# Jun-CEN/Open-World-Semantic-Segmentation

Hardware: AMD Instinct MI355X
Metric: images/sec train-step, DeepLabV3+R101 768x768 bs=16; % HBM & MFMA roofline (higher is better)
Workload: dtype f16x2

## Files before the change

include/dmlnet_hip.h:

```cpp
#ifndef DMLNET_HIP_H
#define DMLNET_HIP_H

#include <stdint.h>

#ifdef __cplusplus
extern "C" {
#endif

#define DML_ABI_VERSION 6

enum { DML_F32 = 0, DML_BF16 = 1 };
enum { DML_EINVAL = -1, DML_EALIGN = -2, DML_EUNSUPPORTED = -3 };

int dml_abi_version(void);
const char* dml_target_arch(void);

typedef struct DmlConvDesc {
    const void* x;
    const void* w;
    void* y;
    const float* bias;
    float* stats;
    int32_t B, Hi, Wi, C, ldx;
    int32_t Ho, Wo, N, ldy;
// ... 106 lines not shown
                    float* scale, float* shift, float* save_mean, float* save_invstd, void* stream);
int dml_bn_moments(float* partials, int64_t M, int N, int stat_rows, double* moments, void* stream);
int dml_bn_finalize_moments(const double* moments, int ranks, int64_t M_each, int N, const float* gamma,
                            const float* beta, float* running_mean, float* running_var, float momentum,
                            float eps, float* scale, float* shift, float* save_mean, float* save_invstd,
                            void* stream);
int dml_bn_bwd_sums(float* partials, int nblocks, int N, double* sums, float* dgamma, float* dbeta,
                    void* stream);
int dml_bn_bwd_coef(const double* sums, int64_t M_total, int N, const float* gamma, const float* save_mean,
                    const float* save_invstd, float* coef, void* stream);
int dml_bn_stats(const void* y, float* partials, int64_t M, int N, int ldy, int dtype, void* stream);
int dml_bn_eval_coeffs(const float* gamma, const float* beta, const float* running_mean,
                       const float* running_var, float eps, float* scale, float* shift, int N,
                       void* stream);
typedef struct DmlBnEvalDesc {
    const float* gamma; const float* beta; const float* running_var; float* scale; float* shift;
    int32_t N; float eps;
} DmlBnEvalDesc;
int dml_bn_eval_coeffs_table(const DmlBnEvalDesc* table, int count, void* stream);
int dml_bn_apply(const void* y, const void* res, void* z, const float* scale, const float* shift,
                 const float* mean, uint8_t* mask, int64_t M, int N, int ldy, int ldres, int ldz, int relu,
                 int dtype, float drop_p, uint64_t drop_seed, float* amax, void* planes, int64_t plane_stride,
                 int32_t ldp, const float* unscale, int64_t res_plane_stride, const float* res_unscale, void* stream);
int dml_bn_bwd_reduce(const void* dz, const void* y, const void* z, const uint8_t* mask, const float* save_mean,
                      const float* save_invstd, float* partials, int64_t M, int N, int lddz, int ldy,
                      int ldz, int relu, float gscale, int dtype, int* nblocks, float* gmax, void* stream);
int dml_bn_bwd_finalize(float* partials, int nblocks, int64_t M, int N, const float* gamma,
                        const float* save_mean, const float* save_invstd, float* dgamma, float* dbeta,
                        float* coef, void* stream);
int dml_bn_bwd_apply(const void* dz, const void* y, const void* z, const uint8_t* mask, const float* coef, void* dy,
                     void* dres, int64_t M, int N, int lddz, int ldy, int ldz, int lddy, int lddres,
                     int relu, float gscale, int dres_accum, int dtype, float* amax, void* planes, int64_t plane_stride,
                     int32_t ldp, const float* unscale, void* stream);
int dml_h2_bound_bn(const float* gamma, const float* beta, int N, int64_t count, float mult, const float* res_amax,
                    float* work, void* stream);
int dml_h2_bound_bn_bwd(const float* coef, const float* save_invstd, int N, int64_t count, const float* g_amax,
                        float* work, void* stream);
int dml_bn_finalize_bound(float* partials, int64_t M, int N, int stat_rows, const float* gamma, const float* beta,
                          float* running_mean, float* running_var, float momentum, float eps,
                          float* scale, float* shift, float* save_mean, float* save_invstd,
                          int64_t count, float mult, const float* res_amax, float* work, uint32_t* state, void* stream);
int dml_bn_bwd_finalize_bound(float* partials, int nblocks, int64_t M, int N, const float* gamma,
                              const float* save_mean, const float* save_invstd, float* dgamma, float* dbeta,
                              float* coef, int64_t count, const float* g_amax, float* work, uint32_t* state, void* stream);
typedef struct DmlH2BoundDesc {
    const float* gamma;
    const float* beta;
    float* work;
    int32_t N;
    float root_count, mult;
    int32_t reserved;
} DmlH2BoundDesc;
int dml_h2_bound_bn_table(const DmlH2BoundDesc* table_device, int count, void* stream);
int dml_h2_bound_bn_multi(const DmlH2BoundDesc* table_device, int count, float* work, void* stream);

int dml_maxpool3x3s2_fwd(const void* x, void* y, uint8_t* argmax, int B, int H, int W, int C, int dtype,
                         void* stream);
int dml_maxpool3x3s2_bwd(const void* dy, const uint8_t* argmax, void* dx, int B, int H, int W, int C,
                         int dtype, void* stream);
int dml_global_avgpool_fwd(const void* x, void* y, int B, int HW, int C, int ldx, int dtype, void* stream);
int dml_broadcast_hw(const void* v, void* z, int B, int HW, int C, int ldz, int dtype, void* stream);
int dml_reduce_hw(const void* dz, void* dv, int B, int HW, int C, int lddz, int dtype, void* stream);
int dml_reduce_hw_f32(const void* x, float* out, int B, int HW, int C, int ldx, int dtype, float scale, void* stream);
int dml_avgpool_bwd_add(const void* dv, void* dx, int B, int HW, int C, int lddx, int dtype, void* stream);
int dml_avgpool_bwd_set(const void* dv, void* dx, int B, int HW, int C, int lddx, int dtype, void* stream);

// ... 127 lines not shown
```

open-world-semantic-segmentation_amd/csrc/bn.hip:

```cpp
#include "common.h"
#include <cstdlib>

namespace {

struct Moments {
    double n, mean, m2;
};
__device__ __forceinline__ void merge(Moments& a, double nb, double meanb, double m2b) {
    if (nb <= 0.0) return;
    const double n = a.n + nb;
    const double d = meanb - a.mean;
    a.mean += d * (nb / n);
    a.m2 += m2b + d * d * (a.n * nb / n);
    a.n = n;
}

constexpr int FIN_CH = 4, FIN_SL = 64;
__device__ __forceinline__ double shfl_xor_f64(double v, int mask) {
    const long long b = __double_as_longlong(v);
    const int lo = __shfl_xor((int)(b & 0xffffffffll), mask), hi = __shfl_xor((int)(b >> 32), mask);
    return __longlong_as_double(((long long)hi << 32) | (unsigned int)lo);
}

__device__ __forceinline__ float h2_words_max(const float* __restrict__ words, float* sh4) {
// ... 647 lines not shown
                    rb[u] = *reinterpret_cast<const float4*>(dres + m * lddres + c + 4);
                }
            }
        }
#pragma unroll
        for (int u = 0; u < U; ++u) {
            const int64_t m = m0 + (int64_t)u * RB;
            if (m >= r1) continue;
            float g[V] = {ga[u].x, ga[u].y, ga[u].z, ga[u].w, gb[u].x, gb[u].y, gb[u].z, gb[u].w};
            const float yy[V] = {ya[u].x, ya[u].y, ya[u].z, ya[u].w, yb[u].x, yb[u].y, yb[u].z, yb[u].w};
#pragma unroll
            for (int q = 0; q < V; ++q) {
                const bool on = ((bits[u] >> (q + (q >= 4 ? 4 : 0))) & 1u) != 0;
                g[q] = on ? g[q] : 0.f;
            }
            h8 hi, lo;
#pragma unroll
            for (int q = 0; q < V; ++q) {
                const float o = cA[q] * g[q] + cB[q] * (yy[q] - cM[q]) + cC[q];
                const float xs = o * h2s;
                const _Float16 h = (_Float16)xs;
                hi[q] = h;
                lo[q] = (_Float16)(xs - (float)h);
            }
            *reinterpret_cast<h8*>(planes + m * ldp + c) = hi;
            *reinterpret_cast<h8*>(planes + plane_stride + m * ldp + c) = lo;
            if (dres != nullptr) {
                float r[V] = {0.f, 0.f, 0.f, 0.f, 0.f, 0.f, 0.f, 0.f};
                if (dres_accum) { r[0] = ra[u].x; r[1] = ra[u].y; r[2] = ra[u].z; r[3] = ra[u].w; r[4] = rb[u].x; r[5] = rb[u].y; r[6] = rb[u].z; r[7] = rb[u].w; }
#pragma unroll
                for (int q = 0; q < V; ++q) r[q] += g[q] * gscale;
                *reinterpret_cast<float4*>(dres + m * lddres + c) = make_float4(r[0], r[1], r[2], r[3]);
                *reinterpret_cast<float4*>(dres + m * lddres + c + 4) = make_float4(r[4], r[5], r[6], r[7]);
            }
        }
    }
}

constexpr int FIN2_MAXCHUNK = 128;
__global__ __launch_bounds__(256) void bn_fold_partials_kernel(float* partials, int64_t G, int N, int R, int NC,
                                                               int last_rows, const int SR) {
    __shared__ double sh[3][4][64];
    const int c = threadIdx.x & 63, rl = threadIdx.x >> 6;
    const int n = blockIdx.x * 64 + c;
    const int64_t g0 = (int64_t)blockIdx.y * R;
    const int64_t g1 = (int)blockIdx.y == NC - 1 ? G : g0 + R;
    double S = 0.0, Q = 0.0, P = 0.0;
    if (n < N)
        #pragma unroll 8
        for (int64_t g = g0 + rl; g < g1; g += 4) {
            const float2 p = *reinterpret_cast<const float2*>(partials + (g * N + n) * 2);
            const double rows = g == G - 1 ? (double)last_rows : (double)SR;
            S += (double)p.x;
            Q += (double)p.y;
            P += (double)p.x * (double)p.x / rows;
        }
    sh[0][rl][c] = S;
    sh[1][rl][c] = Q;
    sh[2][rl][c] = P;
    __syncthreads();
    if (rl < 3 && n < N) {
        const double v = sh[rl][0][c] + sh[rl][1][c] + sh[rl][2][c] + sh[rl][3][c];
        reinterpret_cast<double*>(partials)[(g0 + rl) * N + n] = v;
    }
}

// ... 298 lines not shown
extern "C" int dml_bn_finalize_moments(const double* moments, int ranks, int64_t M_each, int N, const float* gamma,
                                       const float* beta, float* running_mean, float* running_var, float momentum,
                                       float eps, float* scale, float* shift, float* save_mean, float* save_invstd,
                                       void* stream) {
    if (!moments || !scale || !shift || !save_mean || ranks <= 0 || M_each <= 0 || N <= 0) return DML_EINVAL;
    hipLaunchKernelGGL(bn_finalize_moments_kernel, dim3((N + 255) / 256), dim3(256), 0, static_cast<hipStream_t>(stream),
                       moments, ranks, M_each, N, gamma, beta, running_mean, running_var, momentum, eps, scale, shift,
                       save_mean, save_invstd);
    DML_LAUNCH_CHECK();
    return 0;
}

extern "C" int dml_bn_bwd_sums(float* partials, int nblocks, int N, double* sums, float* dgamma, float* dbeta,
                               void* stream) {
    if (!partials || !sums || nblocks <= 0 || N <= 0) return DML_EINVAL;
    hipStream_t st = static_cast<hipStream_t>(stream);
    const int stride = fold_bwd_partials(partials, nblocks, N, st);
    hipLaunchKernelGGL(bn_bwd_finalize_kernel, dim3((N + FIN_CH - 1) / FIN_CH), dim3(256), 0, st, partials, nblocks,
                       (int64_t)1, N, (const float*)nullptr, (const float*)nullptr, (const float*)nullptr, dgamma, dbeta,
                       (float*)nullptr, sums, stride);
    DML_LAUNCH_CHECK();
    return 0;
}

extern "C" int dml_bn_bwd_coef(const double* sums, int64_t M_total, int N, const float* gamma, const float* save_mean,
                               const float* save_invstd, float* coef, void* stream) {
    if (!sums || !save_mean || !save_invstd || !coef || M_total <= 0 || N <= 0) return DML_EINVAL;
    hipLaunchKernelGGL(bn_bwd_coef_kernel, dim3((N + 255) / 256), dim3(256), 0, static_cast<hipStream_t>(stream), sums,
                       M_total, N, gamma, save_mean, save_invstd, coef);
    DML_LAUNCH_CHECK();
    return 0;
}

extern "C" int dml_bn_bwd_apply(const void* dz, const void* y, const void* z, const uint8_t* mask, const float* coef, void* dy,
                                void* dres, int64_t M, int N, int lddz, int ldy, int ldz, int lddy, int lddres,
                                int relu, float gscale, int dres_accum, int dtype, float* amax, void* planes,
                                int64_t plane_stride, int32_t ldp, const float* unscale, void* stream) {
    if (!dz || !y || !coef || (!dy && !planes) || M <= 0 || N <= 0) return DML_EINVAL;
    if (relu && !z && !mask) return DML_EINVAL;
    if (!vec_ok(dtype, N) || !vec_ok(dtype, lddz) || !vec_ok(dtype, ldy) || (dy && !vec_ok(dtype, lddy)) ||
        (relu && !mask && !vec_ok(dtype, ldz)) || (dres && !vec_ok(dtype, lddres)))
        return DML_EALIGN;
    if (M >= (1ll << 31)) return DML_EINVAL;
    if (planes) {
        if (dtype != DML_F32 || !unscale || plane_stride <= 0 || ldp < N) return DML_EINVAL;
        if ((ldp & 3) || (plane_stride & 3) || (reinterpret_cast<uintptr_t>(planes) & 7)) return DML_EALIGN;
    }
    const int V = dtype == DML_BF16 ? 8 : 4;
    hipStream_t st = static_cast<hipStream_t>(stream);
    constexpr int bt = 64;
    if (dtype == DML_F32 && planes && !dy && !amax && (mask || !relu) && (N & 7) == 0 && (lddz & 3) == 0 && (ldy & 3) == 0 &&
        (ldp & 7) == 0 && (plane_stride & 7) == 0 && (!dres || (lddres & 3) == 0) &&
        ((reinterpret_cast<uintptr_t>(planes) | reinterpret_cast<uintptr_t>(dz) | reinterpret_cast<uintptr_t>(y) |
          reinterpret_cast<uintptr_t>(dres)) & 15) == 0 && (reinterpret_cast<uintptr_t>(mask) & 1) == 0) {
        const ColGeom g8 = col_geom(M, N / 8, 2, stream_blocks(M, N, dtype), bt);
        hipLaunchKernelGGL((bn_bwd_apply_planes8_kernel<2>), dim3(g8.row_blocks, g8.col_chunks), dim3(bt), 0, st, (const float*)dz,
                           (const float*)y, mask, coef, (float*)dres, M, N, lddz, ldy, lddres, relu, gscale, dres_accum, g8.CB, g8.RB,
                           g8.rows_per_block, static_cast<_Float16*>(planes), plane_stride, (int)ldp, unscale);
        DML_LAUNCH_CHECK();
        return 0;
    }
    const ColGeom g = col_geom(M, N / V, 2, stream_blocks(M, N, dtype), bt);
    dim3 grid(g.row_blocks, g.col_chunks);
    if (dtype == DML_BF16)
        hipLaunchKernelGGL((bn_bwd_apply_cols_kernel<bf16_t, 2>), grid, dim3(bt), 0, st, (const bf16_t*)dz,
                           (const bf16_t*)y, (const bf16_t*)z, mask, coef, (bf16_t*)dy, (bf16_t*)dres, M, N, lddz, ldy,
                           ldz, lddy, lddres, relu, gscale, dres_accum, g.CB, g.RB, g.rows_per_block,
                           reinterpret_cast<uint32_t*>(amax), (_Float16*)nullptr, (int64_t)0, 0, (const float*)nullptr);
    else
        hipLaunchKernelGGL((bn_bwd_apply_cols_kernel<float, 2>), grid, dim3(bt), 0, st, (const float*)dz,
                           (const float*)y, (const float*)z, mask, coef, (float*)dy, (float*)dres, M, N, lddz, ldy, ldz,
                           lddy, lddres, relu, gscale, dres_accum, g.CB, g.RB, g.rows_per_block, reinterpret_cast<uint32_t*>(amax),
                           static_cast<_Float16*>(planes), plane_stride, (int)ldp, unscale);
    DML_LAUNCH_CHECK();
    return 0;
}

namespace {
__global__ __launch_bounds__(256) void h2_bound_kernel(const float* __restrict__ p0, const float* __restrict__ p1,
                                                       const float* __restrict__ p2, const float* __restrict__ invstd, int N,
                                                       float root_count, float mult, const float* __restrict__ words,
                                                       float* __restrict__ work, int bwd) {
    __shared__ float sh[4];
    __shared__ uint32_t shw[4];
    uint32_t wm = 0;
    if (words != nullptr)
        for (int i = threadIdx.x; i < 1024; i += 256) wm = max(wm, __float_as_uint(words[i]));
#pragma unroll
    for (int o = 32; o > 0; o >>= 1) wm = max(wm, (uint32_t)__shfl_xor((int)wm, o, 64));
    if ((threadIdx.x & 63) == 0) shw[threadIdx.x >> 6] = wm;
    __syncthreads();
    const float wmax = __uint_as_float(max(max(shw[0], shw[1]), max(shw[2], shw[3])));
    float b = 0.f;
    for (int n = threadIdx.x; n < N; n += 256) {
        float v;
        if (!bwd) v = fabsf(p0 ? p0[n] : 1.f) * root_count + fabsf(p1 ? p1[n] : 0.f);
        else v = fabsf(p0[n]) * wmax + fabsf(p1[n]) * root_count / invstd[n] + fabsf(p2[n]);
        b = fmaxf(b, v);
    }
#pragma unroll
    for (int o = 32; o > 0; o >>= 1) b = fmaxf(b, __shfl_xor(b, o, 64));
    if ((threadIdx.x & 63) == 0) sh[threadIdx.x >> 6] = b;
    __syncthreads();
    if (threadIdx.x != 0) return;
    b = fmaxf(fmaxf(sh[0], sh[1]), fmaxf(sh[2], sh[3]));
    b = bwd ? b : b * mult + wmax;
    b *= 1.0009765625f;
    const uint32_t m = __float_as_uint(b);
    float s = 1.0f;
    if (m != 0) {
// ... 88 lines not shown
```

open-world-semantic-segmentation_amd/csrc/plan_exec.hip:

```cpp
#include "common.h"

#include <cstring>
#include <tuple>
#include <utility>

namespace {

template <class T> struct Unpack {
    static T get(uint64_t w) {
        if constexpr (std::is_pointer<T>::value) {
            return reinterpret_cast<T>(static_cast<uintptr_t>(w));
        } else if constexpr (std::is_same<T, float>::value) {
            const uint32_t lo = (uint32_t)w;
            float f;
            std::memcpy(&f, &lo, 4);
            return f;
        } else if constexpr (std::is_same<T, double>::value) {
            double d;
            std::memcpy(&d, &w, 8);
            return d;
        } else {
            return static_cast<T>(static_cast<int64_t>(w));
        }
    }
// ... 12 lines not shown
struct Entry {
    const char* name;
    int (*run)(const uint64_t*, void*);
    int nargs;
};

#define DML_ENTRY(fn) {#fn, [](const uint64_t* w, void* st) -> int { return thunk_call(&fn, w, st); }, arity(&fn)}

const Entry kEntries[] = {
    DML_ENTRY(dml_conv_igemm),
    DML_ENTRY(dml_conv_wgrad),
    DML_ENTRY(dml_conv_wgrad_group),
    DML_ENTRY(dml_prep_weight),
    DML_ENTRY(dml_prep_weights),
    DML_ENTRY(dml_unpad_wgrad),
    DML_ENTRY(dml_bias_grad),
    DML_ENTRY(dml_bias_grad_ws),
    DML_ENTRY(dml_pack_input),
    DML_ENTRY(dml_pack_input_s2d),
    DML_ENTRY(dml_s2d_weights),
    DML_ENTRY(dml_s2d_wgrad),
    DML_ENTRY(dml_bn_finalize),
    DML_ENTRY(dml_bn_moments),
    DML_ENTRY(dml_bn_finalize_moments),
    DML_ENTRY(dml_bn_bwd_sums),
    DML_ENTRY(dml_bn_bwd_coef),
    DML_ENTRY(dml_bn_stats),
    DML_ENTRY(dml_bn_eval_coeffs),
    DML_ENTRY(dml_bn_eval_coeffs_table),
    DML_ENTRY(dml_bn_apply),
    DML_ENTRY(dml_bn_bwd_reduce),
    DML_ENTRY(dml_bn_bwd_finalize),
    DML_ENTRY(dml_bn_bwd_apply),
    DML_ENTRY(dml_maxpool3x3s2_fwd),
    DML_ENTRY(dml_maxpool3x3s2_bwd),
    DML_ENTRY(dml_global_avgpool_fwd),
    DML_ENTRY(dml_broadcast_hw),
    DML_ENTRY(dml_reduce_hw),
    DML_ENTRY(dml_reduce_hw_f32),
    DML_ENTRY(dml_avgpool_bwd_add),
    DML_ENTRY(dml_avgpool_bwd_set),
    DML_ENTRY(dml_bilinear_fwd),
    DML_ENTRY(dml_bilinear_bwd),
    DML_ENTRY(dml_proto_dist_fwd),
    DML_ENTRY(dml_upsample_dist_fwd),
    DML_ENTRY(dml_proto_dist_bwd),
    DML_ENTRY(dml_head_bwd_fused),
    DML_ENTRY(dml_argmax_msp),
    DML_ENTRY(dml_dissum_score),
    DML_ENTRY(dml_novel_relabel),
    DML_ENTRY(dml_loss_fwd),
    DML_ENTRY(dml_loss_finalize),
    DML_ENTRY(dml_loss_bwd),
    DML_ENTRY(dml_sgd_step),
    DML_ENTRY(dml_fill_f32),
    DML_ENTRY(dml_convert_dtype),
    DML_ENTRY(dml_adaptive_avgpool_fwd),
    DML_ENTRY(dml_proto_dist_nhwc),
    DML_ENTRY(dml_upsample_nhwc_to_nchw),
    DML_ENTRY(dml_confusion_update),
    DML_ENTRY(dml_class_feature_sum),
    DML_ENTRY(dml_label_encode),
    DML_ENTRY(dml_h2_split),
    DML_ENTRY(dml_h2_bound_bn),
    DML_ENTRY(dml_h2_bound_bn_bwd),
    DML_ENTRY(dml_h2_bound_bn_table),
// ... 97 lines not shown
```

open-world-semantic-segmentation_amd/dmlnet/_lib.py:

```python
from __future__ import annotations

import ctypes as C
import os

_HERE = os.path.dirname(os.path.abspath(__file__))
LIB_PATH = os.environ.get("DML_LIB_PATH") or os.path.join(_HERE, "libdmlnet_hip.so")

DML_F32, DML_BF16 = 0, 1
STAT_ROWS = 64
LOSS_BLOCKS = 2048

c_p = C.c_void_p
c_i = C.c_int
c_i64 = C.c_int64
c_f = C.c_float


class ConvDesc(C.Structure):
    _fields_ = [("x", c_p), ("w", c_p), ("y", c_p), ("bias", c_p), ("stats", c_p),
                ("B", C.c_int32), ("Hi", C.c_int32), ("Wi", C.c_int32), ("C", C.c_int32), ("ldx", C.c_int32),
                ("Ho", C.c_int32), ("Wo", C.c_int32), ("N", C.c_int32), ("ldy", C.c_int32),
                ("R", C.c_int32), ("S", C.c_int32), ("stride", C.c_int32), ("dil", C.c_int32),
                ("pad", C.c_int32), ("dtype", C.c_int32), ("y_f32", C.c_int32), ("accum", C.c_int32),
                ("mode", C.c_int32),
# ... 73 lines not shown
_PROTOS = {
    "dml_abi_version": (c_i, []),
    "dml_target_arch": (C.c_char_p, []),
    "dml_conv_igemm": (c_i, [C.POINTER(ConvDesc), c_p]),
    "dml_conv_stat_rows": (c_i, [C.POINTER(ConvDesc)]),
    "dml_h2_split_table": (c_i, [c_p, c_i, c_p]),
    "dml_h2_split": (c_i, [c_p, c_i64, c_i, c_i, c_p, c_i64, c_i, c_i, c_p, c_i, c_p]),
    "dml_conv_wgrad": (c_i, [C.POINTER(WgradDesc), c_p]),
    "dml_prep_weight": (c_i, [c_p, c_p, c_p, c_i, c_i, c_i, c_i, c_i, c_p]),
    "dml_prep_weights": (c_i, [c_p, c_i, c_i, c_p]),
    "dml_unpad_wgrad": (c_i, [c_p, c_p, c_i, c_i, c_i, c_i, c_p]),
    "dml_bias_grad": (c_i, [c_p, c_p, c_i64, c_i, c_i, c_i, c_p]),
    "dml_bias_grad_ws": (c_i, [c_p, c_p, c_i64, c_i, c_i, c_i, c_p, c_i64, c_p]),
    "dml_pack_input": (c_i, [c_p, c_p, c_i, c_i, c_i, c_i, c_i, c_i, c_p]),
    "dml_pack_input_s2d": (c_i, [c_p, c_p, c_i, c_i, c_i, c_i, c_p]),
    "dml_s2d_weights": (c_i, [c_p, c_p, c_i, c_i, c_i, c_p]),
    "dml_s2d_wgrad": (c_i, [c_p, c_p, c_i, c_i, c_i, c_p]),
    "dml_gather_taps": (c_i, [c_p, c_p, c_i, c_i, c_i, c_i, c_i, c_i, c_i, c_i, c_p]),
    "dml_bn_finalize": (c_i, [c_p, c_i64, c_i, c_i, c_p, c_p, c_p, c_p, c_f, c_f, c_p, c_p, c_p, c_p, c_p]),
    "dml_bn_moments": (c_i, [c_p, c_i64, c_i, c_i, c_p, c_p]),
    "dml_bn_finalize_moments": (c_i, [c_p, c_i, c_i64, c_i, c_p, c_p, c_p, c_p, c_f, c_f, c_p, c_p, c_p, c_p, c_p]),
    "dml_bn_bwd_sums": (c_i, [c_p, c_i, c_i, c_p, c_p, c_p, c_p]),
    "dml_bn_bwd_coef": (c_i, [c_p, c_i64, c_i, c_p, c_p, c_p, c_p, c_p]),
    "dml_bn_stats": (c_i, [c_p, c_p, c_i64, c_i, c_i, c_i, c_p]),
    "dml_bn_eval_coeffs": (c_i, [c_p, c_p, c_p, c_p, c_f, c_p, c_p, c_i, c_p]),
    "dml_bn_eval_coeffs_table": (c_i, [c_p, c_i, c_p]),
    "dml_bn_apply": (c_i, [c_p, c_p, c_p, c_p, c_p, c_p, c_p, c_i64, c_i, c_i, c_i, c_i, c_i, c_i, c_f, C.c_uint64, c_p,
                           c_p, c_i64, c_i, c_p, c_i64, c_p, c_p]),
    "dml_bn_bwd_reduce": (c_i, [c_p, c_p, c_p, c_p, c_p, c_p, c_p, c_i64, c_i, c_i, c_i, c_i, c_i, c_f, c_i,
                                C.POINTER(c_i), c_p, c_p]),
    "dml_bn_bwd_finalize": (c_i, [c_p, c_i, c_i64, c_i, c_p, c_p, c_p, c_p, c_p, c_p, c_p]),
    "dml_bn_bwd_apply": (c_i, [c_p, c_p, c_p, c_p, c_p, c_p, c_p, c_i64, c_i, c_i, c_i, c_i, c_i, c_i, c_i, c_f,
                               c_i, c_i, c_p, c_p, c_i64, c_i, c_p, c_p]),
    "dml_h2_bound_bn": (c_i, [c_p, c_p, c_i, c_i64, c_f, c_p, c_p, c_p]),
    "dml_h2_bound_bn_table": (c_i, [c_p, c_i, c_p]),
    "dml_h2_bound_bn_multi": (c_i, [c_p, c_i, c_p, c_p]),
    "dml_bilinear_fwd_planes": (c_i, [c_p, c_p, c_i64, c_i, c_p, c_i, c_i, c_i, c_i, c_i, c_i, c_i, c_p]),
    "dml_h2_bound_bn_bwd": (c_i, [c_p, c_p, c_i, c_i64, c_p, c_p, c_p]),
    "dml_bn_finalize_bound": (c_i, [c_p, c_i64, c_i, c_i, c_p, c_p, c_p, c_p, c_f, c_f, c_p, c_p, c_p, c_p,
                                    c_i64, c_f, c_p, c_p, c_p, c_p]),
    "dml_bn_bwd_finalize_bound": (c_i, [c_p, c_i, c_i64, c_i, c_p, c_p, c_p, c_p, c_p, c_p, c_i64, c_p, c_p, c_p, c_p]),
    "dml_maxpool3x3s2_fwd": (c_i, [c_p, c_p, c_p, c_i, c_i, c_i, c_i, c_i, c_p]),
    "dml_maxpool3x3s2_bwd": (c_i, [c_p, c_p, c_p, c_i, c_i, c_i, c_i, c_i, c_p]),
    "dml_global_avgpool_fwd": (c_i, [c_p, c_p, c_i, c_i, c_i, c_i, c_i, c_p]),
    "dml_broadcast_hw": (c_i, [c_p, c_p, c_i, c_i, c_i, c_i, c_i, c_p]),
    "dml_reduce_hw": (c_i, [c_p, c_p, c_i, c_i, c_i, c_i, c_i, c_p]),
    "dml_reduce_hw_f32": (c_i, [c_p, c_p, c_i, c_i, c_i, c_i, c_i, c_f, c_p]),
    "dml_avgpool_bwd_add": (c_i, [c_p, c_p, c_i, c_i, c_i, c_i, c_i, c_p]),
    "dml_avgpool_bwd_set": (c_i, [c_p, c_p, c_i, c_i, c_i, c_i, c_i, c_p]),
    "dml_bilinear_fwd": (c_i, [c_p, c_p, c_i, c_i, c_i, c_i, c_i, c_i, c_i, c_i, c_i, c_i, c_i, c_p]),
    "dml_bilinear_bwd": (c_i, [c_p, c_p, c_i, c_i, c_i, c_i, c_i, c_i, c_i, c_i, c_i, c_i, c_i, c_p]),
    "dml_proto_dist_fwd": (c_i, [c_p, c_p, c_p, c_p, c_p, c_p, c_i, c_i, c_i, c_i, c_i, c_p]),
    "dml_upsample_dist_fwd": (c_i, [c_p, c_p, c_p, c_p, c_p, c_p, c_i, c_i, c_i, c_i, c_i, c_i, c_i, c_p]),
    "dml_proto_dist_bwd": (c_i, [c_p, c_p, c_p, c_p, c_p, c_i, c_i, c_i, c_i, c_i, c_p]),
    "dml_head_bwd_fused": (c_i, [c_p, c_p, c_p, c_p, c_p, c_p, c_i, c_i, c_i, c_i, c_i, c_i, c_i, c_i64, c_f, c_f, c_i, c_p]),
    "dml_argmax_msp": (c_i, [c_p, c_p, c_p, c_i, c_i, c_i, c_i, c_p]),
    "dml_dissum_score": (c_i, [c_p, c_p, c_p, c_i, c_i, c_i, c_i, c_f, c_i, c_p]),
    "dml_novel_relabel": (c_i, [c_p, c_p, c_p, c_p, c_i, c_i, c_i, c_i, c_i, c_f, c_i64, c_p]),
    "dml_loss_fwd": (c_i, [c_p, c_p, c_p, c_p, c_i, c_i, c_i, c_i, c_i64, c_p]),
    "dml_loss_finalize": (c_i, [c_p, c_p, c_f, c_f, c_p]),
    "dml_loss_bwd": (c_i, [c_p, c_p, c_p, c_p, c_p, c_i, c_i, c_i, c_i, c_i64, c_f, c_f, c_p]),
    "dml_sgd_step": (c_i, [c_p, c_p, c_p, c_i64, c_f, c_f, c_f, c_f, c_p]),
    "dml_fill_f32": (c_i, [c_p, c_i64, c_f, c_p]),
    "dml_convert_dtype": (c_i, [c_p, c_p, c_i64, c_i, c_i, c_p]),
    "dml_confusion_update": (c_i, [c_p, c_p, c_p, c_i64, c_i, c_p]),
    "dml_class_feature_sum": (c_i, [c_p, c_p, c_i64, c_i, c_i64, c_p, c_p, c_p]),
# ... 60 lines not shown
```

open-world-semantic-segmentation_amd/dmlnet/engine.py:

```python
from __future__ import annotations

import ctypes as C
import itertools
import os
import struct
import weakref
from typing import List, Optional

import numpy as np
import torch
import torch.distributed as dist
import torch.nn as nn

from . import _lib, lazy_grad
from ._lib import DML_BF16, DML_F32, STAT_ROWS, ConvDesc, WgradDesc

_PAD_CIN = 8


class _S2DConv:

    def __init__(self, conv: nn.Conv2d, Ho: int, Wo: int):
        k, p = conv.kernel_size[0], conv.padding[0]
        self.real, self.k = conv, k
# ... 828 lines not shown
            sp = part.data_ptr()
        else:
            sp = self.sp
            a1 = self.call(self.bwd, lib.dml_bn_bwd_reduce, dz.ptr, u.y.ptr, u.z.ptr, mk, u.mean.data_ptr(),
                           u.invstd.data_ptr(), self.sp, M, N, dz.ld, u.y.ld, u.z.ld, 1 if relu_eff else 0, 1.0,
                           self.dt, C.byref(nblk), gwork.data_ptr() if gwork is not None else None)
        if self.sync and not u.frozen:
            sums = self.dbuf(N * 2)
            self.call(self.bwd, lib.dml_bn_bwd_sums, sp, nblk, N, sums.data_ptr(), st.grad_ptr_of(bn.weight),
                      st.grad_ptr_of(bn.bias))
            grp = self.e.sync_group
            self.py_op(self.bwd, lambda t=sums, g=grp: dist.all_reduce(t, group=g))
            self.call(self.bwd, lib.dml_bn_bwd_coef, sums.data_ptr(), M * self.world, N, bn.weight.data_ptr(),
                      u.mean.data_ptr(), u.invstd.data_ptr(), coef.data_ptr())
        elif dy_direct and self.fuse_bound:
            self.call(self.bwd, lib.dml_bn_bwd_finalize_bound, sp, nblk, 0 if u.frozen else M, N, bn.weight.data_ptr(),
                      u.mean.data_ptr(), u.invstd.data_ptr(), st.grad_ptr_of(bn.weight),
                      st.grad_ptr_of(bn.bias), coef.data_ptr(), M * self.world, gwork.data_ptr(), dy.h2[1].data_ptr(),
                      self.bound_state())
            bound_done = True
        else:
            self.call(self.bwd, lib.dml_bn_bwd_finalize, sp, nblk, 0 if u.frozen else M, N, bn.weight.data_ptr(),
                      u.mean.data_ptr(), u.invstd.data_ptr(), st.grad_ptr_of(bn.weight),
                      st.grad_ptr_of(bn.bias), coef.data_ptr())
        self.mark_grad(bn.weight)
        self.mark_grad(bn.bias)
        pl = (None, 0, 0, None)
        if dy_direct:
            planes, work = dy.h2
            if not bound_done:
                self.call(self.bwd, lib.dml_h2_bound_bn_bwd, coef.data_ptr(), u.invstd.data_ptr(), N, M * self.world,
                          gwork.data_ptr(), work.data_ptr())
            pl = (planes.data_ptr(), M * N, N, work.data_ptr() + 4096)
        a3 = self.call(self.bwd, lib.dml_bn_bwd_apply, dz.ptr, u.y.ptr, u.z.ptr, mk, coef.data_ptr(),
                       None if only else dy.ptr, dres.ptr if dres is not None else None, M, N, dz.ld, u.y.ld, u.z.ld, dy.ld,
                       dres.ld if dres is not None else 0, 1 if relu_eff else 0, 1.0,
                       1 if dres_accum else 0, self.dt, None if dy_direct else self.amax_of(dy), *pl)
        u.gscale_slots += ([(a1, 13)] if a1 is not None else []) + [(a3, 15)]
        if dres is not None:
            self.last_dgrad.pop(dres.ptr, None)
        self.conv_wgrad(u.x, dy, u.conv, u.Cp)
        if need_dgrad:
            self.conv_dgrad(dy, u.conv, u.wt, u.x, final=final)

    def block_fwd(self, x: Act, blk: nn.Module, out_planes_only=False):
        n1, n2, n3 = blk.conv1.out_channels, blk.conv2.out_channels, blk.conv3.out_channels
        kk = blk.conv2.kernel_size[0] * blk.conv2.kernel_size[1]
        u1 = self.cbr(x, blk.conv1, blk.bn1, planes_only=self.h2_ok(n1, n2, kk))
        u2 = self.cbr(u1.z, blk.conv2, blk.bn2, planes_only=self.h2_ok(n2, n3, 1))
        ud = None
        if blk.downsample is not None:
            ud = self.cbr(x, blk.downsample[0], blk.downsample[1], relu=False)
            idt = ud.z
        else:
            idt = x
        u3 = self.cbr(u2.z, blk.conv3, blk.bn3, relu=True, res=idt, planes_only=out_planes_only)
        return (x, u1, u2, u3, ud)

    def block_bwd(self, rec):
        xb, u1, u2, u3, ud = rec
        dz = self.grad_of(u3.z)
        ud_from_dz = False
        if ud is not None:
            ud_from_dz = (self.ds_grad_from_dz and u3.relu and u3.mask is not None and u3.drop is None and not ud.relu
                          and ud.drop is None and ud.z is ud.z.root and ud.conv.out_channels == u3.conv.out_channels)
            if ud_from_dz:
                self.unit_bwd(u3, dz, dres=None)
            else:
                dres = self.grad_of(ud.z)
                self.unit_bwd(u3, dz, dres=dres, dres_accum=False)
                ud.z.grad_init = True
        elif (self.fuse_res_grad and not xb.root.grad_init and xb is xb.root
              and u3.relu and u3.mask is not None and u3.drop is None and xb.C % 8 == 0 and xb.C > 32
              and dz.ld == xb.C and self.conv_geom(u1.conv, xb)[:3] == (1, 1, 1)
              and (self.dtype == torch.bfloat16
# ... 216 lines not shown
    def _head_bwd(self, rec, low: Act, out: Act):
        lib, st = self.lib, self.e.store
        B, H, W = self.B, self.H, self.W
        K, Kp, emb, fin, wt_fin = rec.K, rec.Kp, rec.emb, rec.fin, rec.wt_fin
        cat1, cat2, up_low, branches, pooled, upool = rec.cat1, rec.cat2, rec.up_low, rec.branches, rec.pooled, rec.upool
        uproj, ucls = rec.uproj, rec.ucls
        df = self.fbuf(B * H * W * Kp)
        rec.df = df
        de = self.new(B, emb.H, emb.W, Kp)
        rec.de = de
        rec.fused_args, rec.fused_range = None, None
        if Kp == 16 and K == 16 and H == 4 * emb.H and W == 4 * emb.W:
            i0 = len(self.bwd)
            rec.fused_args = self.call(self.bwd, lib.dml_head_bwd_fused, 0, 0, 0, 0, rec.protos.data_ptr(), de.ptr, B,
                                       emb.H, emb.W, Kp, K, H, W, 255, 0.0, 1.0, self.dt)
            rec.fused_range = (i0, i0 + 1)
        i1 = len(self.bwd)
        rec.head_bwd_args = self.call(self.bwd, lib.dml_proto_dist_bwd, 0, None, 0, rec.protos.data_ptr(),
                                       df.data_ptr(), B, Kp, K, H, W)
        self.call(self.bwd, lib.dml_bilinear_bwd, df.data_ptr(), de.ptr, B, emb.H, emb.W, H, W, Kp, Kp, Kp, self.dt, 1, 0)
        rec.unfused_range = (i1, i1 + 2)
        if fin.bias is not None:
            bws = self.fbuf(1024 * Kp)
            if Kp == K:
                self.call(self.bwd, lib.dml_bias_grad_ws, de.ptr, st.grad_ptr_of(fin.bias), de.M, K, de.ld, self.dt,
                          bws.data_ptr(), bws.numel())
            else:
                gb = self.fbuf(Kp)
                self.call(self.bwd, lib.dml_fill_f32, gb.data_ptr(), Kp, 0.0)
                self.call(self.bwd, lib.dml_bias_grad_ws, de.ptr, gb.data_ptr(), de.M, Kp, de.ld, self.dt, bws.data_ptr(),
                          bws.numel())
                self.call(self.bwd, lib.dml_unpad_wgrad, gb.data_ptr(), st.grad_ptr_of(fin.bias), 1, 1, K, Kp)
            self.mark_grad(fin.bias)
        self.conv_wgrad(ucls.z, de, fin, 256, pad_rows=Kp)
        self.conv_dgrad(de, fin, wt_fin, ucls.z)
        self.unit_bwd(ucls, self.grad_of(ucls.z))
        dcat2 = self.grad_of(cat2)
        dproj = self.grad_of(uproj.z)
        self.call(self.bwd, lib.dml_bilinear_bwd, dcat2.slice(48, 256).ptr, dproj.ptr, B, out.H, out.W, low.H, low.W,
                  256, dcat2.ld, dproj.ld, self.dt, 0, 0)
        uproj.z.grad_init = True
        self.unit_bwd(uproj, dproj)
        dcat1 = self.grad_of(cat1)
        staged = out.g32 is not None
        if rec.pool_f32:
            with self.precision(torch.float32):
                dzp = self.new(B, 1, 1, 256)
                self.call(self.bwd, lib.dml_reduce_hw_f32, dcat1.slice(1024, 256).ptr, dzp.ptr, B, out.H * out.W, 256,
                          dcat1.ld, DML_BF16, 1.0)
                self.unit_bwd(upool, dzp)
                gp32 = self.grad_of(pooled)
            if not staged:
                gpq = self.new(B, 1, 1, out.C)
                self.call(self.bwd, lib.dml_convert_dtype, gp32.ptr, gpq.ptr, B * out.C, DML_F32, DML_BF16)
        else:
            assert not staged
            dzp = self.new(B, 1, 1, 256)
            self.call(self.bwd, lib.dml_reduce_hw, dcat1.slice(1024, 256).ptr, dzp.ptr, B, out.H * out.W, 256, dcat1.ld,
                      self.dt)
            self.unit_bwd(upool, dzp)
            gpq = self.grad_of(pooled)
        feeders = self.to_backbone_ops
        first = not out.root.grad_init
        if staged:
            self.call(self.bwd, lib.dml_avgpool_bwd_set if first else lib.dml_avgpool_bwd_add, gp32.ptr, out.g32.ptr, B,
                      out.H * out.W, out.C, out.g32.ld, DML_F32)
        else:
            self.call(self.bwd, lib.dml_avgpool_bwd_set if first else lib.dml_avgpool_bwd_add, gpq.ptr,
# ... 223 lines not shown
        self._exec(self.fwd, stream, pos, len(self.fwd))

    @staticmethod
    def run(ops, stream, start=0, stop=None, hook=None, skipped=()):
        stop = len(ops) if stop is None else stop
        for i in range(start, stop):
            if i in skipped:
                if hook is not None:
                    hook(i)
                continue
            fn, args = ops[i]
            rc = fn(*args, stream)
            if rc:
                _lib.check(rc, getattr(fn, "__name__", "kernel") + " (op %d)" % i)
            if hook is not None:
                hook(i)

    _py_run = run


class Engine:

    plan_cls = Plan

    def __init__(self, model: nn.Module):
        self.model = model
        self.lib = _lib.load()
        self.store = ParamStore(model)
        self.plans = {}
        self._protos = {}
        self.reducer = None
        self.overlap_wgrad = os.environ.get("DML_OVERLAP_WGRAD", "1") != "0"
        self.native = os.environ.get("DML_NATIVE_PLAN", "1") != "0"
        self.sync_bn, self.sync_group = False, None
        self.f32_split = {"exact": 0, "bf16x3": 1, "f16x2": 2}[os.environ.get("DML_F32_PRODUCTS", "exact").lower()]
        self._side = {}
        self._branch = {}
        self.step_count = 0
        self.seed = 0x5DEECE66D

    def rank_seed(self) -> int:
        rank = dist.get_rank() if (dist.is_available() and dist.is_initialized()) else 0
        return (self.seed ^ (rank * 0xD1B54A32D192ED03)) & 0xFFFFFFFFFFFFFFFF

    def side_stream(self, device):
        if device not in self._side:
            self._side[device] = torch.cuda.Stream(device=device)
        return self._side[device]

    def branch_streams(self, device, n):
        pool = self._branch.setdefault(device, [])
        while len(pool) < n:
            pool.append(torch.cuda.Stream(device=device))
        return pool[:n]

    def prototypes(self, k: int) -> torch.Tensor:
        dev = self.store.flat_p.device
        key = (k, dev)
        if key not in self._protos:
            self._protos[key] = 3.0 * torch.eye(k, dtype=torch.float32, device=dev)
        return self._protos[key]

    def head_modules(self):
        m = self.model
        return m.head_modules() if hasattr(m, "head_modules") else [m.classifier]

# ... 152 lines not shown
```

Baseline: 211.7.

## Issue dgrad before wgrad and add lean 4-wide BN backward apply kernel

Reorders backward so each conv's data-gradient is launched before its weight-gradient, letting the critical-path dgrad proceed while wgrad overlaps on the side stream. Adds a lean BN-backward-apply kernel that works on 4-wide vectors with 32-bit byte offsets, 64-thread blocks and a fixed waves-per-EU hint, aiming to cut address arithmetic and register pressure. The lean path is used only when wgrad overlap is enabled and the offsets fit in 32 bits. Narrower vectors could cost memory-transaction efficiency, and the reordering shifts stream scheduling.

```diff
diff --git a/include/dmlnet_hip.h b/include/dmlnet_hip.h
--- a/include/dmlnet_hip.h
+++ b/include/dmlnet_hip.h
@@ -162,6 +162,10 @@
                      void* dres, int64_t M, int N, int lddz, int ldy, int ldz, int lddy, int lddres,
                      int relu, float gscale, int dres_accum, int dtype, float* amax, void* planes, int64_t plane_stride,
                      int32_t ldp, const float* unscale, void* stream);
+int dml_bn_bwd_apply_lean(const void* dz, const void* y, const void* z, const uint8_t* mask, const float* coef, void* dy,
+                          void* dres, int64_t M, int N, int lddz, int ldy, int ldz, int lddy, int lddres,
+                          int relu, float gscale, int dres_accum, int dtype, float* amax, void* planes, int64_t plane_stride,
+                          int32_t ldp, const float* unscale, void* stream);
 int dml_h2_bound_bn(const float* gamma, const float* beta, int N, int64_t count, float mult, const float* res_amax,
                     float* work, void* stream);
 int dml_h2_bound_bn_bwd(const float* coef, const float* save_invstd, int N, int64_t count, const float* g_amax,
diff --git a/open-world-semantic-segmentation_amd/csrc/bn.hip b/open-world-semantic-segmentation_amd/csrc/bn.hip
--- a/open-world-semantic-segmentation_amd/csrc/bn.hip
+++ b/open-world-semantic-segmentation_amd/csrc/bn.hip
@@ -703,6 +703,81 @@
                 for (int q = 0; q < V; ++q) r[q] += g[q] * gscale;
                 *reinterpret_cast<float4*>(dres + m * lddres + c) = make_float4(r[0], r[1], r[2], r[3]);
                 *reinterpret_cast<float4*>(dres + m * lddres + c + 4) = make_float4(r[4], r[5], r[6], r[7]);
+            }
+        }
+    }
+}
+
+template <int U, bool ACC>
+__global__ __launch_bounds__(64) __attribute__((amdgpu_waves_per_eu(6, 6))) void bn_bwd_apply_planes4_lean_kernel(
+    const float* __restrict__ dz, const float* __restrict__ y, const uint8_t* __restrict__ mask, const float* __restrict__ coef,
+    float* dres, int M, int N, int lddz, int ldy, int lddres, int relu, float gscale, int CB, int RB,
+    int rows_per_block, _Float16* __restrict__ planes, uint32_t plane_bytes, int ldp, const float* __restrict__ unscale) {
+    typedef _Float16 h4 __attribute__((ext_vector_type(4)));
+    constexpr int V = 4;
+    const float h2s = 1.0f / unscale[0];
+    const int NV = N / V;
+    const int col = threadIdx.x % CB, rl = threadIdx.x / CB;
+    const int vcol = blockIdx.y * CB + col;
+    if (!(rl < RB && vcol < NV)) return;
+    const int c = vcol * V;
+    float cA[V], cB[V], cC[V], cM[V];
+#pragma unroll
+    for (int q = 0; q < V; ++q) {
+        cA[q] = coef[c + q] * gscale;
+        cB[q] = coef[N + c + q];
+        cC[q] = coef[2 * N + c + q];
+        cM[q] = coef[3 * N + c + q];
+    }
+    const char* dzb = reinterpret_cast<const char*>(dz);
+    const char* yb = reinterpret_cast<const char*>(y);
+    char* rb = reinterpret_cast<char*>(dres);
+    char* pb = reinterpret_cast<char*>(planes);
+    const int r0 = blockIdx.x * rows_per_block;
+    const int r1 = min(M, r0 + rows_per_block);
+    for (int m0 = r0 + rl; m0 < r1; m0 += RB * U) {
+        float4 g4[U], y4[U], r4[U];
+        uint32_t bits[U];
+#pragma unroll
+        for (int u = 0; u < U; ++u) {
+            const int m = m0 + u * RB;
+            bits[u] = 0xfu;
+            if (m < r1) {
+                g4[u] = *reinterpret_cast<const float4*>(dzb + ((uint32_t)(m * lddz + c) << 2));
+                y4[u] = *reinterpret_cast<const float4*>(yb + ((uint32_t)(m * ldy + c) << 2));
+                if (relu) bits[u] = mask[(uint32_t)(m * NV + vcol)];
+                if (ACC) r4[u] = *reinterpret_cast<const float4*>(rb + ((uint32_t)(m * lddres + c) << 2));
+            }
+        }
+#pragma unroll
+        for (int u = 0; u < U; ++u) {
+            const int m = m0 + u * RB;
+            if (m >= r1) continue;
+            float g[V] = {g4[u].x, g4[u].y, g4[u].z, g4[u].w};
+            const float yy[V] = {y4[u].x, y4[u].y, y4[u].z, y4[u].w};
+#pragma unroll
+            for (int q = 0; q < V; ++q) {
+                const bool on = ((bits[u] >> q) & 1u) != 0;
+                g[q] = on ? g[q] : 0.f;
+            }
+            h4 hi, lo;
+#pragma unroll
+            for (int q = 0; q < V; ++q) {
+                const float o = cA[q] * g[q] + cB[q] * (yy[q] - cM[q]) + cC[q];
+                const float xs = o * h2s;
+                const _Float16 h = (_Float16)xs;
+                hi[q] = h;
+                lo[q] = (_Float16)(xs - (float)h);
+            }
+            const uint32_t po = (uint32_t)(m * ldp + c) << 1;
+            *reinterpret_cast<h4*>(pb + po) = hi;
+            *reinterpret_cast<h4*>(pb + plane_bytes + po) = lo;
+            if (dres != nullptr) {
+                float r[V] = {0.f, 0.f, 0.f, 0.f};
+                if (ACC) { r[0] = r4[u].x; r[1] = r4[u].y; r[2] = r4[u].z; r[3] = r4[u].w; }
+#pragma unroll
+                for (int q = 0; q < V; ++q) r[q] += g[q] * gscale;
+                *reinterpret_cast<float4*>(rb + ((uint32_t)(m * lddres + c) << 2)) = make_float4(r[0], r[1], r[2], r[3]);
             }
         }
     }
@@ -1067,10 +1142,10 @@
     return 0;
 }
 
-extern "C" int dml_bn_bwd_apply(const void* dz, const void* y, const void* z, const uint8_t* mask, const float* coef, void* dy,
-                                void* dres, int64_t M, int N, int lddz, int ldy, int ldz, int lddy, int lddres,
-                                int relu, float gscale, int dres_accum, int dtype, float* amax, void* planes,
-                                int64_t plane_stride, int32_t ldp, const float* unscale, void* stream) {
+static int bn_bwd_apply_launch(const void* dz, const void* y, const void* z, const uint8_t* mask, const float* coef, void* dy,
+                               void* dres, int64_t M, int N, int lddz, int ldy, int ldz, int lddy, int lddres,
+                               int relu, float gscale, int dres_accum, int dtype, float* amax, void* planes,
+                               int64_t plane_stride, int32_t ldp, const float* unscale, void* stream, const bool lean) {
     if (!dz || !y || !coef || (!dy && !planes) || M <= 0 || N <= 0) return DML_EINVAL;
     if (relu && !z && !mask) return DML_EINVAL;
     if (!vec_ok(dtype, N) || !vec_ok(dtype, lddz) || !vec_ok(dtype, ldy) || (dy && !vec_ok(dtype, lddy)) ||
@@ -1088,6 +1163,22 @@
         (ldp & 7) == 0 && (plane_stride & 7) == 0 && (!dres || (lddres & 3) == 0) &&
         ((reinterpret_cast<uintptr_t>(planes) | reinterpret_cast<uintptr_t>(dz) | reinterpret_cast<uintptr_t>(y) |
           reinterpret_cast<uintptr_t>(dres)) & 15) == 0 && (reinterpret_cast<uintptr_t>(mask) & 1) == 0) {
+        const int64_t ldmax = std::max<int64_t>(std::max(lddz, ldy), dres ? lddres : 0);
+        if (lean && M * ldmax < (1ll << 30) && 2 * (plane_stride + M * ldp) < (1ll << 32)) {
+            const bool acc = dres && dres_accum;
+            const ColGeom g4 = col_geom(M, N / 4, acc ? 2 : 3, stream_blocks(M, N, dtype), bt);
+            const dim3 grid(g4.row_blocks, g4.col_chunks);
+            if (acc)
+                hipLaunchKernelGGL((bn_bwd_apply_planes4_lean_kernel<2, true>), grid, dim3(bt), 0, st, (const float*)dz, (const float*)y,
+                                   mask, coef, (float*)dres, (int)M, N, lddz, ldy, lddres, relu, gscale, g4.CB, g4.RB, g4.rows_per_block,
+                                   static_cast<_Float16*>(planes), (uint32_t)(2 * plane_stride), (int)ldp, unscale);
+            else
+                hipLaunchKernelGGL((bn_bwd_apply_planes4_lean_kernel<3, false>), grid, dim3(bt), 0, st, (const float*)dz, (const float*)y,
+                                   mask, coef, (float*)dres, (int)M, N, lddz, ldy, lddres, relu, gscale, g4.CB, g4.RB, g4.rows_per_block,
+                                   static_cast<_Float16*>(planes), (uint32_t)(2 * plane_stride), (int)ldp, unscale);
+            DML_LAUNCH_CHECK();
+            return 0;
+        }
         const ColGeom g8 = col_geom(M, N / 8, 2, stream_blocks(M, N, dtype), bt);
         hipLaunchKernelGGL((bn_bwd_apply_planes8_kernel<2>), dim3(g8.row_blocks, g8.col_chunks), dim3(bt), 0, st, (const float*)dz,
                            (const float*)y, mask, coef, (float*)dres, M, N, lddz, ldy, lddres, relu, gscale, dres_accum, g8.CB, g8.RB,
@@ -1111,6 +1202,22 @@
     return 0;
 }
 
+extern "C" int dml_bn_bwd_apply(const void* dz, const void* y, const void* z, const uint8_t* mask, const float* coef, void* dy,
+                                void* dres, int64_t M, int N, int lddz, int ldy, int ldz, int lddy, int lddres,
+                                int relu, float gscale, int dres_accum, int dtype, float* amax, void* planes,
+                                int64_t plane_stride, int32_t ldp, const float* unscale, void* stream) {
+    return bn_bwd_apply_launch(dz, y, z, mask, coef, dy, dres, M, N, lddz, ldy, ldz, lddy, lddres, relu, gscale, dres_accum, dtype, amax,
+                               planes, plane_stride, ldp, unscale, stream, false);
+}
+
+extern "C" int dml_bn_bwd_apply_lean(const void* dz, const void* y, const void* z, const uint8_t* mask, const float* coef, void* dy,
+                                     void* dres, int64_t M, int N, int lddz, int ldy, int ldz, int lddy, int lddres,
+                                     int relu, float gscale, int dres_accum, int dtype, float* amax, void* planes,
+                                     int64_t plane_stride, int32_t ldp, const float* unscale, void* stream) {
+    return bn_bwd_apply_launch(dz, y, z, mask, coef, dy, dres, M, N, lddz, ldy, ldz, lddy, lddres, relu, gscale, dres_accum, dtype, amax,
+                               planes, plane_stride, ldp, unscale, stream, true);
+}
+
 namespace {
 __global__ __launch_bounds__(256) void h2_bound_kernel(const float* __restrict__ p0, const float* __restrict__ p1,
                                                        const float* __restrict__ p2, const float* __restrict__ invstd, int N,
diff --git a/open-world-semantic-segmentation_amd/csrc/plan_exec.hip b/open-world-semantic-segmentation_amd/csrc/plan_exec.hip
--- a/open-world-semantic-segmentation_amd/csrc/plan_exec.hip
+++ b/open-world-semantic-segmentation_amd/csrc/plan_exec.hip
@@ -68,6 +68,7 @@
     DML_ENTRY(dml_bn_bwd_reduce),
     DML_ENTRY(dml_bn_bwd_finalize),
     DML_ENTRY(dml_bn_bwd_apply),
+    DML_ENTRY(dml_bn_bwd_apply_lean),
     DML_ENTRY(dml_maxpool3x3s2_fwd),
     DML_ENTRY(dml_maxpool3x3s2_bwd),
     DML_ENTRY(dml_global_avgpool_fwd),
diff --git a/open-world-semantic-segmentation_amd/dmlnet/_lib.py b/open-world-semantic-segmentation_amd/dmlnet/_lib.py
--- a/open-world-semantic-segmentation_amd/dmlnet/_lib.py
+++ b/open-world-semantic-segmentation_amd/dmlnet/_lib.py
@@ -129,6 +129,8 @@
     "dml_bn_bwd_finalize": (c_i, [c_p, c_i, c_i64, c_i, c_p, c_p, c_p, c_p, c_p, c_p, c_p]),
     "dml_bn_bwd_apply": (c_i, [c_p, c_p, c_p, c_p, c_p, c_p, c_p, c_i64, c_i, c_i, c_i, c_i, c_i, c_i, c_i, c_f,
                                c_i, c_i, c_p, c_p, c_i64, c_i, c_p, c_p]),
+    "dml_bn_bwd_apply_lean": (c_i, [c_p, c_p, c_p, c_p, c_p, c_p, c_p, c_i64, c_i, c_i, c_i, c_i, c_i, c_i, c_i, c_f,
+                                    c_i, c_i, c_p, c_p, c_i64, c_i, c_p, c_p]),
     "dml_h2_bound_bn": (c_i, [c_p, c_p, c_i, c_i64, c_f, c_p, c_p, c_p]),
     "dml_h2_bound_bn_table": (c_i, [c_p, c_i, c_p]),
     "dml_h2_bound_bn_multi": (c_i, [c_p, c_i, c_p, c_p]),
diff --git a/open-world-semantic-segmentation_amd/dmlnet/engine.py b/open-world-semantic-segmentation_amd/dmlnet/engine.py
--- a/open-world-semantic-segmentation_amd/dmlnet/engine.py
+++ b/open-world-semantic-segmentation_amd/dmlnet/engine.py
@@ -884,15 +884,18 @@
                 self.call(self.bwd, lib.dml_h2_bound_bn_bwd, coef.data_ptr(), u.invstd.data_ptr(), N, M * self.world,
                           gwork.data_ptr(), work.data_ptr())
             pl = (planes.data_ptr(), M * N, N, work.data_ptr() + 4096)
-        a3 = self.call(self.bwd, lib.dml_bn_bwd_apply, dz.ptr, u.y.ptr, u.z.ptr, mk, coef.data_ptr(),
+        apply = lib.dml_bn_bwd_apply_lean if self.e.overlap_wgrad and self.e.lean_bn_bwd else lib.dml_bn_bwd_apply
+        a3 = self.call(self.bwd, apply, dz.ptr, u.y.ptr, u.z.ptr, mk, coef.data_ptr(),
                        None if only else dy.ptr, dres.ptr if dres is not None else None, M, N, dz.ld, u.y.ld, u.z.ld, dy.ld,
                        dres.ld if dres is not None else 0, 1 if relu_eff else 0, 1.0,
                        1 if dres_accum else 0, self.dt, None if dy_direct else self.amax_of(dy), *pl)
         u.gscale_slots += ([(a1, 13)] if a1 is not None else []) + [(a3, 15)]
         if dres is not None:
             self.last_dgrad.pop(dres.ptr, None)
+        if need_dgrad and self.e.dgrad_first:
+            self.conv_dgrad(dy, u.conv, u.wt, u.x, final=final)
         self.conv_wgrad(u.x, dy, u.conv, u.Cp)
-        if need_dgrad:
+        if need_dgrad and not self.e.dgrad_first:
             self.conv_dgrad(dy, u.conv, u.wt, u.x, final=final)
 
     def block_fwd(self, x: Act, blk: nn.Module, out_planes_only=False):
@@ -1175,8 +1178,11 @@
                           bws.numel())
                 self.call(self.bwd, lib.dml_unpad_wgrad, gb.data_ptr(), st.grad_ptr_of(fin.bias), 1, 1, K, Kp)
             self.mark_grad(fin.bias)
+        if self.e.dgrad_first:
+            self.conv_dgrad(de, fin, wt_fin, ucls.z)
         self.conv_wgrad(ucls.z, de, fin, 256, pad_rows=Kp)
-        self.conv_dgrad(de, fin, wt_fin, ucls.z)
+        if not self.e.dgrad_first:
+            self.conv_dgrad(de, fin, wt_fin, ucls.z)
         self.unit_bwd(ucls, self.grad_of(ucls.z))
         dcat2 = self.grad_of(cat2)
         dproj = self.grad_of(uproj.z)
@@ -1466,6 +1472,8 @@
         self.reducer = None
         self.overlap_wgrad = os.environ.get("DML_OVERLAP_WGRAD", "1") != "0"
         self.native = os.environ.get("DML_NATIVE_PLAN", "1") != "0"
+        self.dgrad_first = True
+        self.lean_bn_bwd = True
         self.sync_bn, self.sync_group = False, None
         self.f32_split = {"exact": 0, "bf16x3": 1, "f16x2": 2}[os.environ.get("DML_F32_PRODUCTS", "exact").lower()]
         self._side = {}
```

Result: slower. 207.7 (-1.9%).
